# nlesc-smcm/hymls

Measured on AMD Instinct MI355X. Metric: Preconditioner ApplyInverse DoF/s + achieved HBM GB/s, Stokes3D, higher is better.
Workload: dtype f64

## Files before the change

### hymls_amd/csrc/device.hpp

```cpp
#pragma once
#include <cstdio>
#include "common.hpp"
#include "symbolic.hpp"

namespace hymls {
namespace dev {

struct Context;
Context* create_context(int device);
void bind(Context* c);
Context* current();
void destroy_context(Context* c);
void* stream();
const double* zeros16();
void* alloc(size_t bytes);
void free(void* p);
void h2d(void* dst, const void* src, size_t bytes);
void d2h(void* dst, const void* src, size_t bytes);
void d2d(void* dst, const void* src, size_t bytes);
void zero(void* dst, size_t bytes);
void sync();
size_t mem_free();
void* shared_scratch(size_t bytes);
constexpr int NSIDE = 8;
// ... 52 lines not shown
  const int32_t* fw_ptr;
  const int32_t* fw_items;
  const struct FwRec* fw_rec;
  const int32_t* bw_ptr;
  const int32_t* bw_items;
  int32_t nlev, max_level_rows;
  int32_t s_ent_begin, s_ent_end;
  int64_t scratch_size, factor_size;
  int32_t contrib_size;
  int32_t max_solve_rows;
  int32_t packed;
};

struct BatchD {
  int32_t nb;
  const int32_t* src;
  const int32_t* xoff;
  double* factor;
  double* scratch;
  double* sblock;
  double* contrib;
  int32_t* flag;
  double* tmp;
  int64_t tmp_stride;
  double* swork;
  int64_t swork_stride;
};

void gather(int64_t n, const int32_t* idx, const double* src, double* dst);
void scatter(int64_t n, const int32_t* idx, const double* src, double* dst);
void scatter_add(int64_t n, const int32_t* idx, const double* src, double* dst);
void axpby(int64_t n, double a, const double* x, double b, double* y);
void scale_copy(int64_t n, double a, const double* x, double* y);
void spmv(int32_t nrows, const int32_t* rowptr, const int32_t* col, const double* val,
          const double* x, double* y, double alpha, double beta, int64_t nnz_hint = -1);
void pull_sum(int64_t n, const int64_t* ptr, const int64_t* idx, const double* in, double* out);
void offdiag_count(int64_t nrows, const int32_t* rows, const int32_t* krow, const int32_t* kcol, const int32_t* ta, const int32_t* tb,
                   const int32_t* excl, int32_t* count);
void offdiag_fill(int64_t nrows, const int32_t* rows, const int32_t* krow, const int32_t* kcol, const int32_t* ta, const int32_t* tb,
                  const int32_t* excl, const int32_t* rowptr, int32_t* col, int32_t* src);
void member_sources(int32_t nb, int32_t next, int32_t nent, const int32_t* ext, const int32_t* ent_row, const int32_t* ent_col,
                    const int32_t* krow, const int32_t* kcol, int32_t* src, int32_t* flag);
void build_pull_tables(int64_t nrows, const int64_t* rcount, const int32_t* rowptr, const uint64_t* keys, int64_t* ptr, int64_t* idx);
void pull_sum_blocks(int64_t blen, int32_t nblk, const int64_t* ptr, const int64_t* base,
                     const double* in, double* out);

void factor_level(const PlanD& P, const BatchD& B, const int32_t* list, int32_t count,
                  int32_t b0, int32_t nbc, const double* kval, int32_t max_w);
void sblock_init(const PlanD& P, const BatchD& B, int32_t b0, int32_t nbc, const double* kval);

constexpr int PIECE = 128;
void factor_big_front(const PlanD& P, const BatchD& B, const FrontD& F, const FrontD* kids, int32_t nkids,
                      int32_t b0, int32_t nbc, const double* kval);
void root_update(const PlanD& P, const BatchD& B, const FrontD& F, int32_t nbc);
inline int solve_kt() {
  static const int kt = (std::getenv("HYMLS_MI_SOLVE_KT") && std::atoi(std::getenv("HYMLS_MI_SOLVE_KT")) == 1024) ? 1024 : 256;
  return kt;
}
void solve_fwd_big(const PlanD& P, const BatchD& B, const int32_t* list, const FrontD* hfronts, const int64_t* poff,
                   int32_t count, double* x);
void solve_bwd_big(const PlanD& P, const BatchD& B, const int32_t* list, const FrontD* hfronts, const int64_t* poff,
                   int32_t count, double* x);

void solve_fwd_level(const PlanD& P, const BatchD& B, const int32_t* list, int32_t count, double* x);
void solve_bwd_level(const PlanD& P, const BatchD& B, const int32_t* list, int32_t count, double* x);

#if defined(__HIPCC__)
#define HYMLS_HD __host__ __device__
#else
#define HYMLS_HD
#endif
HYMLS_HD inline int64_t packed_lower(int64_t w, int64_t i, int64_t k) { return k * (2 * w - k - 1) / 2 + (i - k - 1); }
HYMLS_HD inline int64_t packed_l21(int64_t w, int64_t ri, int64_t i, int64_t k) { return w * (w - 1) / 2 + i + ri * k; }
HYMLS_HD inline int64_t packed_upper(int64_t w, int64_t ri, int64_t i, int64_t k) { return w * (w - 1) / 2 + ri * w + k * (k + 1) / 2 + i; }
void repack_fronts(const PlanD& P, const BatchD& B, int32_t b0, int32_t nbc);

struct FusedSub {
  union {
    const double* fac;
    const float* fac32;
  };
  int32_t xoff;
  int32_t cls;
};
constexpr int FUSED_MAX_ITEMS = 2048;
struct FusedIO {
  int32_t in = 0, out = 0;
  const double* b = nullptr; const int32_t* perm = nullptr;
  const int32_t* a_row = nullptr; const int32_t* a_col = nullptr; const double* a_val = nullptr; const double* x2 = nullptr;
  const double* z = nullptr; double* user = nullptr;
};
void interior_solve_fused(int32_t nsub, const FusedSub* subs, const PlanD* plans, int32_t lds_doubles, double* x,
                          const FusedIO* io = nullptr);

constexpr int32_t FLAG_F32_RANGE = 4;
void demote_panels(int64_t n, const double* src, float* dst, int32_t* flag);
void round_panels(int64_t n, double* slab, int32_t* flag);
void interior_solve_fused_f32(int32_t nsub, const FusedSub* subs, const PlanD* plans, int32_t lds_doubles, double* x,
                              const FusedIO* io = nullptr);

struct LvlSub { const double* fac; double* contrib; int32_t xoff, cls; int64_t cstride; };
struct LvlTask { int32_t sub, front, r0, pad; };
constexpr int LVL_MAX_ROWS = 6144;
constexpr int LVL_SMALL_ROWS = 256;
void solve_fwd_tasks(const LvlTask* tasks, int32_t ntasks, const LvlSub* subs, const PlanD* plans, int32_t lds_doubles,
                     const double* x, double* y);
void solve_bwd_tasks(const LvlTask* tasks, int32_t ntasks, const LvlSub* subs, const PlanD* plans, int32_t lds_doubles,
                     const double* y, double* x);

constexpr int NV_MAX = 4;
void interior_solve_fused_mv(int32_t nsub, const FusedSub* subs, const PlanD* plans, int32_t lds_doubles, int32_t front_doubles,
                             double* x, int64_t ldx, int nv);
void interior_solve_fused_mv_f32(int32_t nsub, const FusedSub* subs, const PlanD* plans, int32_t lds_doubles, int32_t front_doubles,
                                 double* x, int64_t ldx, int nv);
void solve_fwd_tasks_mv(const LvlTask* tasks, int32_t ntasks, const LvlSub* subs, const PlanD* plans, int32_t lds_doubles,
                        const double* x, double* y, int64_t ld, int nv);
void solve_bwd_tasks_mv(const LvlTask* tasks, int32_t ntasks, const LvlSub* subs, const PlanD* plans, int32_t lds_doubles,
                        const double* y, double* x, int64_t ld, int nv);

void ot_apply(int32_t ng, const int32_t* gptr, const double* w, double* x);
// ... 26 lines not shown
```

### hymls_amd/csrc/device_hip.hip

```cpp
#include <hip/hip_runtime.h>
#include <type_traits>
#include <dlfcn.h>
#include <chrono>
#include <cstring>
#include <cfloat>
#include <array>
#include <map>
#include <string>
#include <cstdio>
#include "device.hpp"

namespace hymls {
namespace dev {

#define HIP_CHECK(call)                                                                    \
  do {                                                                                     \
    hipError_t e_ = (call);                                                                \
    if (e_ != hipSuccess)                                                                  \
      throw ::hymls::Error(-3, std::string("HIP error: ") + hipGetErrorString(e_) + " at " + \
                                   __FILE__ + ":" + std::to_string(__LINE__));             \
  } while (0)

struct MarkRec { int phase; bool begin; hipEvent_t ev; };
struct Context {
// ... 263 lines not shown
  if (n <= 0) return;
  hipLaunchKernelGGL(k_scatter_add, dim3(nblocks(n, 256, 65536)), dim3(256), 0, g_stream, n, idx, src, dst); launch_check();
}
void axpby(int64_t n, double a, const double* x, double b, double* y) {
  if (n <= 0) return;
  hipLaunchKernelGGL(k_axpby, dim3(nblocks(n, 256, 8192)), dim3(256), 0, g_stream, n, a, x, b, y); launch_check();
}
void scale_copy(int64_t n, double a, const double* x, double* y) {
  if (n <= 0) return;
  hipLaunchKernelGGL(k_scale_copy, dim3(nblocks(n, 256, 8192)), dim3(256), 0, g_stream, n, a, x, y); launch_check();
}

template <int L>
__global__ void k_spmv(int32_t nrows, const int32_t* __restrict__ rp, const int32_t* __restrict__ col,
                       const double* __restrict__ val, const double* __restrict__ x, double* __restrict__ y,
                       double alpha, double beta) {
  const int lane = (int)(threadIdx.x % L);
  const int rpb = (int)blockDim.x / L;
  for (int64_t base = (int64_t)blockIdx.x * rpb; base < nrows; base += (int64_t)gridDim.x * rpb) {
    const int64_t row = base + threadIdx.x / L;
    double s = 0.0;
    if (row < nrows) {
      const int b = rp[row], e = rp[row + 1];
      for (int k = b + lane; k < e; k += L) s += val[k] * x[col[k]];
    }
#pragma unroll
    for (int off = L / 2; off > 0; off >>= 1) s += __shfl_down(s, off, L);
    if (row < nrows && lane == 0) y[row] = alpha * s + (beta == 0.0 ? 0.0 : beta * y[row]);
  }
}
void spmv(int32_t nrows, const int32_t* rp, const int32_t* col, const double* val, const double* x, double* y,
          double alpha, double beta, int64_t nnz_hint) {
  if (nrows <= 0) return;
  const double avg = nnz_hint >= 0 ? (double)nnz_hint / nrows : 8.0;
  const int L = avg < 2.5 ? 1 : (avg < 5.0 ? 2 : (avg < 20.0 ? 4 : 8));
  const int64_t nt = (int64_t)nrows * L;
  const dim3 grid(nblocks(nt, 256));
  switch (L) {
    case 1: hipLaunchKernelGGL(k_spmv<1>, grid, dim3(256), 0, g_stream, nrows, rp, col, val, x, y, alpha, beta); break;
    case 2: hipLaunchKernelGGL(k_spmv<2>, grid, dim3(256), 0, g_stream, nrows, rp, col, val, x, y, alpha, beta); break;
    case 4: hipLaunchKernelGGL(k_spmv<4>, grid, dim3(256), 0, g_stream, nrows, rp, col, val, x, y, alpha, beta); break;
    default: hipLaunchKernelGGL(k_spmv<8>, grid, dim3(256), 0, g_stream, nrows, rp, col, val, x, y, alpha, beta); break;
  }
  launch_check();
}

__global__ void k_pull_sum(int64_t n, const int64_t* __restrict__ ptr, const int64_t* __restrict__ idx,
                           const double* __restrict__ in, double* __restrict__ out) {
  for (int64_t e = blockIdx.x * (int64_t)blockDim.x + threadIdx.x; e < n; e += (int64_t)gridDim.x * blockDim.x) {
    double s = 0.0;
    for (int64_t t = ptr[e]; t < ptr[e + 1]; t++) s += in[idx[t]];
    out[e] = s;
  }
}
void pull_sum(int64_t n, const int64_t* ptr, const int64_t* idx, const double* in, double* out) {
  if (n <= 0) return;
  hipLaunchKernelGGL(k_pull_sum, dim3(nblocks(n, 256, 65536)), dim3(256), 0, g_stream, n, ptr, idx, in, out); launch_check();
}
template <bool FILL>
__global__ void __launch_bounds__(256) k_offdiag(int64_t nrows, const int32_t* __restrict__ rows, const int32_t* __restrict__ krow,
                                                 const int32_t* __restrict__ kcol, const int32_t* __restrict__ ta, const int32_t* __restrict__ tb,
                                                 const int32_t* __restrict__ excl, const int32_t* __restrict__ rowptr, int32_t* __restrict__ out,
                                                 int32_t* __restrict__ src) {
  for (int64_t t = blockIdx.x * (int64_t)blockDim.x + threadIdx.x; t < nrows; t += (int64_t)gridDim.x * blockDim.x) {
    const int32_t r = rows[t];
    int32_t o = FILL ? rowptr[t] : 0;
    for (int32_t e = krow[r]; e < krow[r + 1]; e++) {
      const int32_t c = kcol[e];
// ... 1625 lines not shown
  if ((uintptr_t)(src + head) % 16 != 0) head = n;
  hipLaunchKernelGGL(k_demote_panels, dim3(nblocks(std::max<int64_t>(n / 4, 1), 256, 8192)), dim3(256), 0, g_stream, src, dst, n, head, flag);
  launch_check();
}
__global__ void __launch_bounds__(256) k_round_panels(double* __restrict__ slab, int64_t n, int32_t* __restrict__ flag) {
  bool bad = false;
  for (int64_t t = (int64_t)blockIdx.x * 256 + threadIdx.x; t < n; t += (int64_t)gridDim.x * 256) {
    const double v = slab[t];
    bad |= !(fabs(v) <= (double)FLT_MAX);
    slab[t] = (double)(float)v;
  }
  if (bad) atomicOr(flag, FLAG_F32_RANGE);
}
void round_panels(int64_t n, double* slab, int32_t* flag) {
  if (n <= 0) return;
  hipLaunchKernelGGL(k_round_panels, dim3(nblocks(n, 256, 8192)), dim3(256), 0, g_stream, slab, n, flag);
  launch_check();
}

struct FusedFront { int32_t c0, w, ri, c_off, a_off, lf_off, idx_off, pad; int64_t lp_off, q_off; };
template <class PTR>
__device__ inline PTR lside(PTR base, int packed, int r, int w, int ri, int& c1, int& tri) {
  if (!packed) { c1 = w + ri; tri = 0; return base + r; }
  if (r < w) { c1 = w; tri = 1; return base + (r - 1); }
  c1 = ri; tri = 0;
  return base + ((w * (w - 1)) >> 1) + (r - w);
}
template <class PTR>
__device__ inline PTR uside(PTR base, int packed, int i, int w, int ri, int& c1, int& tri) {
  if (!packed) { c1 = w + ri; tri = 0; return base + i; }
  c1 = 0; tri = 1;
  return base + ((w * (w - 1)) >> 1) + ri * w + i;
}
template <bool PROF, class PT>
__global__ void __launch_bounds__(256) __attribute__((amdgpu_waves_per_eu(8, 8))) k_interior_fused(const FusedSub* __restrict__ subs, const PlanD* __restrict__ plans,
                                                         double* __restrict__ x, long long* __restrict__ prof, FusedIO io) {
  extern __shared__ double lds[];
  auto ldp = [](gptr<PT> q) { return (double)*q; };
  long long tp[6] = {0, 0, 0, 0, 0, 0}, t0 = 0, tstart = 0;
  auto tick = [&](int bucket) { if (PROF) { const long long t = wall_clock64(); tp[bucket] += t - t0; t0 = t; } };
  if (PROF) { t0 = wall_clock64(); tstart = t0; }
  const FusedSub S = subs[blockIdx.x];
  const PlanD P = plans[S.cls];
  double* X = lds;
  double* C = lds + P.nI;
  double* Fv = C + P.contrib_size;
  double* R = Fv + 128;
  FusedFront* LF = (FusedFront*)(Fv + (P.max_level_rows > 384 ? P.max_level_rows : 384));
  const int tid = threadIdx.x;
  for (int i = tid; i < P.nfronts; i += 256) {
    const FrontD G = P.fronts[i];
    FusedFront f;
    f.c0 = G.c0; f.w = G.w; f.ri = G.ri; f.c_off = G.c_off; f.a_off = G.a_off; f.lf_off = G.lf_off; f.idx_off = G.idx_off; f.pad = 0;
    f.lp_off = G.lp_off; f.q_off = G.q_off;
    LF[i] = f;
  }
  double* xg = x + S.xoff;
  if (io.in == 0) {
    for (int i = tid; i < P.nI; i += 256) X[i] = xg[i];
  } else if (io.in == 1) {
    for (int i = tid; i < P.nI; i += 256) X[i] = io.b[io.perm[S.xoff + i]];
  } else {
    for (int i = tid; i < P.nI; i += 256) {
      double v = 0.0;
      for (int e = io.a_row[S.xoff + i]; e < io.a_row[S.xoff + i + 1]; e++) v += io.a_val[e] * io.x2[io.a_col[e]];
      X[i] = v;
    }
  }
  __syncthreads();
  tick(0);
  const gptr<PT> fac = as_global((const PT*)(const void*)S.fac);
  const gptr<int32_t> fw_items = as_global(P.fw_items), bw_items = as_global(P.bw_items), fidx = as_global(P.fidx),
                      asm_ptr = as_global(P.asm_ptr), asm_src = as_global(P.asm_src), fw_ptr = as_global(P.fw_ptr), bw_ptr = as_global(P.bw_ptr);
  typedef int v4i __attribute__((ext_vector_type(4)));
  const gptr<v4i> fw_rec = (gptr<v4i>)P.fw_rec;
  for (int lev = 0; lev < P.nlev; lev++) {
    const int ib = fw_ptr[lev], ni = fw_ptr[lev + 1] - ib;
    for (int it = tid; it < ni; it += 256) {
      FwRec rc;
      { const v4i q = fw_rec[ib + it]; static_assert(sizeof(FwRec) == 16, "FwRec is one dwordx4"); __builtin_memcpy(&rc, &q, 16); }
      const int item = rc.item;
      const FusedFront& F = LF[item >> 16];
      const int r = item & 0xffff;
      double v = r < F.w ? X[F.c0 + r] : 0.0;
      if (rc.n != 0xffff) {
#pragma unroll
        for (int q = 0; q < 5; q++) if (q < rc.n) v += C[rc.s[q]];
      } else {
        for (int t = asm_ptr[F.a_off + r]; t < asm_ptr[F.a_off + r + 1]; t++) v += C[asm_src[t]];
      }
      if (r < F.w) Fv[F.lf_off + r] = v; else C[F.c_off + r - F.w] = v;
    }
    __syncthreads();
    tick(1);
    if (ni > 128) {
      for (int it = tid; it < ni; it += 256) {
        const int item = fw_items[ib + it];
        const FusedFront& F = LF[item >> 16];
        const int r = item & 0xffff, w = F.w;
// ... 100 lines not shown
        const int i = item & 0xffff, w = F.w, ri = F.ri;
        int c1, tri;
        const gptr<PT> p = uside(fac + F.lp_off, P.packed, i, w, ri, c1, tri);
        const double* Xs = X + F.c0;
        auto at = [&](int kk) { return ldp(p + (c1 * kk + tri * ((kk * (kk + 1)) >> 1))); };
        int k = i + kg;
        for (; k + 3 * KG < w; k += 4 * KG) {
          const double l0 = at(k), l1 = at(k + KG), l2 = at(k + 2 * KG), l3 = at(k + 3 * KG);
          a0 += l0 * Xs[k]; a1 += l1 * Xs[k + KG]; a2 += l2 * Xs[k + 2 * KG]; a3 += l3 * Xs[k + 3 * KG];
        }
        for (; k < w; k += KG) a0 += at(k) * Xs[k];
        const gptr<PT> qv = fac + F.q_off + i;
        const gptr<int32_t> idx = fidx + F.idx_off + w;
        k = kg;
        for (; k + 3 * KG < ri; k += 4 * KG) {
          const double q0 = ldp(qv + (int64_t)w * k), q1 = ldp(qv + (int64_t)w * (k + KG)), q2 = ldp(qv + (int64_t)w * (k + 2 * KG)), q3 = ldp(qv + (int64_t)w * (k + 3 * KG));
          const int i0 = idx[k], i1 = idx[k + KG], i2 = idx[k + 2 * KG], i3 = idx[k + 3 * KG];
          a0 -= q0 * X[i0]; a1 -= q1 * X[i1]; a2 -= q2 * X[i2]; a3 -= q3 * X[i3];
        }
        for (; k < ri; k += KG) a0 -= ldp(qv + (int64_t)w * k) * X[idx[k]];
      }
      R[kg * RT + it] = (a0 + a1) + (a2 + a3);
      __syncthreads();
      if (tid < ni) {
        const int item = bw_items[ib + tid];
        double sum = 0.0;
        for (int g = 0; g < KG; g++) sum += R[g * RT + tid];
        X[LF[item >> 16].c0 + (item & 0xffff)] = sum;
      }
    }
    __syncthreads();
    tick(ni > 128 ? 3 : 4);
  }
  if (io.out == 0) {
    for (int i = tid; i < P.nI; i += 256) xg[i] = X[i];
  } else {
    for (int i = tid; i < P.nI; i += 256) io.user[io.perm[S.xoff + i]] = io.z[S.xoff + i] - X[i];
  }
  if (PROF && tid == 0) {
    tp[5] = wall_clock64() - tstart;
    for (int q = 0; q < 6; q++) prof[(int64_t)blockIdx.x * 8 + q] = tp[q];
    prof[(int64_t)blockIdx.x * 8 + 6] = tstart;
    prof[(int64_t)blockIdx.x * 8 + 7] = P.nI;
  }
}

template <class PT>
static void launch_fused(int32_t nsub, const FusedSub* subs, const PlanD* plans, int32_t lds_doubles, double* x, const FusedIO* iop) {
  const FusedIO io = iop ? *iop : FusedIO();
  if (nsub <= 0) return;
  const size_t shm = (size_t)lds_doubles * sizeof(double);
  if (std::getenv("HYMLS_MI_FUSED_PROF")) {
    long long* dprof = (long long*)alloc((size_t)nsub * 8 * sizeof(long long));
    if (shm > 64 * 1024) HIP_CHECK(hipFuncSetAttribute((const void*)k_interior_fused<true, PT>, hipFuncAttributeMaxDynamicSharedMemorySize, (int)shm));
    hipLaunchKernelGGL((k_interior_fused<true, PT>), dim3(nsub), dim3(256), shm, g_stream, subs, plans, x, dprof, io);
    launch_check();
    std::vector<long long> h((size_t)nsub * 8);
    d2h(h.data(), dprof, h.size() * sizeof(long long));
    free(dprof);
    double sum[6] = {0, 0, 0, 0, 0, 0};
    long long tmin = h[6], tmax = 0;
    for (int b = 0; b < nsub; b++) { for (int q = 0; q < 6; q++) sum[q] += (double)h[(size_t)b * 8 + q]; tmin = std::min(tmin, h[(size_t)b * 8 + 6]); tmax = std::max(tmax, h[(size_t)b * 8 + 6] + h[(size_t)b * 8 + 5]); }
    std::fprintf(stderr, "[hymls_mi] fused solve: %d workgroups, kernel span %.1f us; mean per workgroup (us): setup %.1f | fwd assembly %.1f | fwd panels %.1f | bwd panels (wide levels) %.1f | bwd panels (k-split levels) %.1f | total %.1f\n",
                 nsub, (tmax - tmin) / 100.0, sum[0] / nsub / 100, sum[1] / nsub / 100, sum[2] / nsub / 100, sum[3] / nsub / 100, sum[4] / nsub / 100, sum[5] / nsub / 100);
    return;
  }
  if (shm > 64 * 1024) HIP_CHECK(hipFuncSetAttribute((const void*)k_interior_fused<false, PT>, hipFuncAttributeMaxDynamicSharedMemorySize, (int)shm));
  hipLaunchKernelGGL((k_interior_fused<false, PT>), dim3(nsub), dim3(256), shm, g_stream, subs, plans, x, (long long*)nullptr, io);
  launch_check();
}
void interior_solve_fused(int32_t nsub, const FusedSub* subs, const PlanD* plans, int32_t lds_doubles, double* x, const FusedIO* iop) {
  launch_fused<double>(nsub, subs, plans, lds_doubles, x, iop);
}
void interior_solve_fused_f32(int32_t nsub, const FusedSub* subs, const PlanD* plans, int32_t lds_doubles, double* x, const FusedIO* iop) {
  launch_fused<float>(nsub, subs, plans, lds_doubles, x, iop);
}

constexpr size_t LDS_LIMIT_BYTES = 160 * 1024;
static int mv_group_cap(const char* which) {
  const char* e = std::getenv((std::string("HYMLS_MI_MV_GROUP_") + which).c_str());
  return e ? std::max(1, std::atoi(e)) : NV_MAX;
}

template <int NV, class PT>
__global__ void __launch_bounds__(256) k_interior_fused_mv(const FusedSub* __restrict__ subs, const PlanD* __restrict__ plans,
                                                            double* __restrict__ x, int64_t ldx) {
  extern __shared__ double lds[];
  const FusedSub S = subs[blockIdx.x];
  const PlanD P = plans[S.cls];
  const int nI = P.nI, CS = P.contrib_size, FS = P.max_level_rows > 384 ? P.max_level_rows : 384;
  double* X = lds;
  double* C = X + NV * nI;
  double* Fv = C + NV * CS;
  FusedFront* LF = (FusedFront*)(Fv + NV * FS);
  const int tid = threadIdx.x;
  for (int i = tid; i < P.nfronts; i += 256) {
    const FrontD G = P.fronts[i];
    FusedFront f;
    f.c0 = G.c0; f.w = G.w; f.ri = G.ri; f.c_off = G.c_off; f.a_off = G.a_off; f.lf_off = G.lf_off; f.idx_off = G.idx_off; f.pad = 0;
    f.lp_off = G.lp_off; f.q_off = G.q_off;
    LF[i] = f;
  }
// ... 1203 lines not shown
```

### hymls_amd/csrc/precond.cpp

```cpp
#include "precond.hpp"
#include <cstring>
#include <chrono>
#include <thread>
#include <mutex>
#include <atomic>
#include <map>
#include <unordered_map>

namespace hymls {

namespace {

struct Hasher {
  uint64_t h = 1469598103934665603ULL;
  void add(const void* p, size_t n) {
    const unsigned char* c = (const unsigned char*)p;
    size_t i = 0;
    for (; i + 8 <= n; i += 8) {
      uint64_t w;
      std::memcpy(&w, c + i, 8);
      h = (h ^ w) * 0x9E3779B97F4A7C15ULL;
      h ^= h >> 29;
    }
    for (; i < n; i++) { h ^= c[i]; h *= 1099511628211ULL; }
// ... 926 lines not shown
      dev::offdiag_fill(nr, d_rows, d_krow_, d_kcol_, ta, tb, excl, d_row, d_col, d_src);
      col.resize(nz); src.resize(nz);
      if (nz) { dev::d2h(col.data(), d_col, nz * sizeof(int32_t)); dev::d2h(src.data(), d_src, nz * sizeof(int32_t)); }
    };
    cut(n1_, d_rows1, d_pos2, nullptr, nullptr, a12_row_, a12_col_, a12_src_, d_a12_row_, d_a12_col_, d_a12_src_);
    fine("A12 count / prefix / fill (device)");
    cut(n2_, d_rows2, d_int, d_ghost, d_pos2, a21_row_, a21_col_, a21_src_, d_a21_row_, d_a21_col_, d_a21_src_);
    dev::sync();
    dev::free(d_pos2); dev::free(d_int); dev::free(d_ghost); dev::free(d_rows1); dev::free(d_rows2);
  }
  if (dist) {
    xch_int_.build(*comm_, want_int, dst_int, [&](int64_t g) { const int l = g2l_[g]; return l >= 0 ? intidx_[l] : -1; });
    xch_sep_.build(*comm_, want_sep, dst_sep, [&](int64_t g) { const int l = g2l_[g]; return (l >= 0 && pos2_[l] < n2_) ? pos2_[l] : -1; });
  }
  fine("A21 count / prefix / fill + halo plans");
  lap("A12/A21 + halo plans");
  for (auto& cp : cls_) {
    const size_t fb = BatchedLU::factor_bytes((int64_t)cp->lu.members.size(), cp->lu.plan.factor_size);
    if (fb >= ((size_t)1 << 30) && !cp->lu.pre_factor) cp->lu.pre_factor.reset(new AsyncAlloc(fb));
  }
  for (auto& cp : cls_) { cp->lu.d_krow = d_krow_; cp->lu.d_kcol = d_kcol_; }
  build_schur_setup();
  lap("Schur setup + uploads");
  d_kval_ = (double*)dev::alloc(std::max<size_t>(1, K_.val.size()) * sizeof(double));
  d_inperm_ = dev::upload(in_perm_);
  d_z_ = (double*)dev::alloc((size_t)std::max(n1_ + ngi_ + n2_, 1) * sizeof(double));
  d_t1_ = (double*)dev::alloc((size_t)std::max(n1_, 1) * sizeof(double));
  d_t2_ = (double*)dev::alloc((size_t)std::max(n2_ + ngs_, 1) * sizeof(double));
  d_y2_ = (double*)dev::alloc((size_t)std::max(n2_, 1) * sizeof(double));
  d_yb_ = (double*)dev::alloc((size_t)std::max(n2_, 1) * sizeof(double));
  d_a12_val_ = (double*)dev::alloc(std::max<size_t>(1, a12_col_.size()) * sizeof(double));
  d_a21_val_ = (double*)dev::alloc(std::max<size_t>(1, a21_col_.size()) * sizeof(double));
  d_flag_ = (int32_t*)dev::alloc(sizeof(int32_t));
  initialized_ = true;
}

void LevelSolver::build_classes() {
  const bool verbose_bc = std::getenv("HYMLS_MI_VERBOSE") != nullptr && (level_ == 0 || std::atoi(std::getenv("HYMLS_MI_VERBOSE")) >= 2);
  double t_bc = wall();
  auto lap_bc = [&](const char* what) {
    if (!verbose_bc) return;
    std::fprintf(stderr, "[hymls_mi] rank %d level %d:   classes / %-22s %.2f s\n", comm_->rank, level_, what, wall() - t_bc);
    t_bc = wall();
  };
  const int n = K_.n;
  const int nsd = (int)hm_.sd.size();
  const int nsep = n2_ + ngs_;
  auto sidx = [&](int32_t gid) { const int l = g2l_[gid]; return l >= 0 ? pos2_[l] : -1; };
  ivec cnt(nsep + 1, 0);
  for (auto& S : hm_.sd) for (auto& g : S.groups) for (int32_t x : g.nodes) { const int k = sidx(x); if (k >= 0) cnt[k + 1]++; }
  for (int i = 0; i < nsep; i++) cnt[i + 1] += cnt[i];
  ivec sdl(cnt[nsep]), fill(cnt.begin(), cnt.end() - 1);
  for (int s = 0; s < nsd; s++)
    for (auto& g : hm_.sd[s].groups) for (int32_t x : g.nodes) { const int k = sidx(x); if (k >= 0) sdl[fill[k]++] = s; }
  auto common = [&](int a, int b) {
    int c = 0, i = cnt[a], j = cnt[b];
    const int ie = cnt[a + 1], je = cnt[b + 1];
    while (i < ie && j < je) {
      const int x = sdl[i], y = sdl[j];
      c += x == y; i += x <= y; j += y <= x;
    }
    return c;
  };
  FineLap fine;
  sep_sd_ptr_ = cnt; sep_sd_ = sdl;
  fine("(classes) subdomains listing each separator node");
// ... 1086 lines not shown
      parallel_assign(next_pattern_key_col_, R.col.data(), R.col.size());
      fnl("(next level) pattern key copy");
      next_level_ = new LevelSolver(p_.next_level(), level_ + 1, ngid_, comm_);
      next_.reset(next_level_);
      next_level_->set_rows(R, next_gids, glob_tv_, R.n);
      fnl("(next level) set_rows");
      next_level_->initialize();
      fnl("(next level) initialize");
      build_handoff(next_level_->owned_gids());
      fnl("(next level) hand-off");
    }
    next_level_->profiling = false;
    lap("next level initialize");
    set_next_border();
    next_level_->set_factor_bits(factor_bits_);
    next_level_->compute();
    lap("next level compute");
  } else {
    DirectSolver* ds = next_is_direct_ && !next_level_ ? dynamic_cast<DirectSolver*>(next_.get()) : nullptr;
    if (!(ds && ds->refactor(R, next_gids, p_.fix_gid, p_, bm_ > 0))) {
      next_.reset();
      next_level_ = nullptr;
      next_is_direct_ = true;
      next_.reset(new DirectSolver(R, next_gids, p_.fix_gid, ngid_, p_, &glob_clu_ptr_, &glob_clu_, &glob_sd_center_, bm_ > 0));
      build_handoff(next_gids);
    }
    set_next_border();
    lap("coarse solver");
  }
}

void LevelSolver::interior_solve(double* x1) { interior_solve_mv(x1, n1_ + ngi_, 1); }

void LevelSolver::interior_solve_mv(double* x1, int64_t ld, int nv) {
  dev::Range range("MatrixBlock", level_ + 1, "ApplyInverse");
  if (n_fsubs_ > 0) {
#ifdef HYMLS_MI_F32_PANELS
    if (fsubs_bits_ == 32) {
      if (nv == 1) dev::interior_solve_fused_f32(n_fsubs_, d_fsubs_, d_fplans_, fused_lds_, x1);
      else dev::interior_solve_fused_mv_f32(n_fsubs_, d_fsubs_, d_fplans_, fused_vec_lds_ + fused_front_lds_, fused_front_lds_, x1, ld, nv);
    } else
#endif
    if (nv == 1) dev::interior_solve_fused(n_fsubs_, d_fsubs_, d_fplans_, fused_lds_, x1);
    else dev::interior_solve_fused_mv(n_fsubs_, d_fsubs_, d_fplans_, fused_vec_lds_ + fused_front_lds_, fused_front_lds_, x1, ld, nv);
  }
  if (merged_.nsubs > 0) {
    ensure_nvec(nv);
    merged_.solve(d_fplans_, x1, d_ytmp_, ld, nv);
  }
  for (size_t c = 0; c < cls_.size(); c++)
    if (!cls_fused_[c] && !cls_merged_[c])
      for (int v = 0; v < nv; v++) cls_[c]->lu.solve(x1 + v * ld);
}

void LevelSolver::ensure_nvec(int nv) {
  if (nv <= nvec_alloc_) return;
  dev::sync();
  auto grow = [&](double*& p, int64_t len) { dev::free(p); p = (double*)dev::alloc((size_t)std::max<int64_t>(len, 1) * nv * sizeof(double)); };
  grow(d_z_, n1_ + ngi_ + n2_); grow(d_t1_, n1_); grow(d_t2_, n2_ + ngs_);
  if (!direct_schur_) { const int64_t ng = (int64_t)vs_.size(); grow(d_vrhs_, ng); grow(d_vsol_, ng); }
  if (d_nrhs_) { grow(d_nrhs_, n_next_owned_); grow(d_nsol_, n_next_owned_); }
  if (d_ytmp_) grow(d_ytmp_, n1_ + ngi_ + n2_);
  nvec_alloc_ = nv;
}

void LevelSolver::next_apply(const double* rhs, double* sol, int64_t ld, int nv) {
  if (!comm_->distributed()) { next_->apply_inverse_mv(rhs, ld, sol, ld, nv); return; }
  const int64_t ldn = std::max<int64_t>(n_next_owned_, 1);
  for (int v = 0; v < nv; v++) xch_down_.forward(rhs + v * ld, d_nrhs_ + v * ldn);
  next_->apply_inverse_mv(d_nrhs_, ldn, d_nsol_, ldn, nv);
  for (int v = 0; v < nv; v++) {
    if (next_is_direct_) {
      if (red_.n) dev::d2d(sol + v * ld, d_nsol_ + v * ldn + glob_row_off_[comm_->rank], (size_t)red_.n * sizeof(double));
    } else {
      xch_down_.backward(d_nsol_ + v * ldn, sol + v * ld);
    }
// ... 1 lines not shown
}

void LevelSolver::schur_apply(double* rhs2, int64_t ldr, double* x2, int64_t ldx, int nv) {
  dev::Range range("SchurPreconditioner", level_ + 1, "ApplyInverse");
  if (global_n2_ == 0) return;
  if (direct_schur_) {
    if (!comm_->distributed()) { next_->apply_inverse_mv(rhs2, ldr, x2, ldx, nv); return; }
    for (int v = 0; v < nv; v++) next_apply(rhs2 + v * ldr, x2 + v * ldx, 0, 1);
    return;
  }
  const int ng = (int)vs_.size();
  const int64_t ldv = std::max(ng, 1);
  for (int v = 0; v < nv; v++) dev::ot_apply(ng, d_gptr_, d_otw_, rhs2 + v * ldr);
  dev::blocks_apply_all_mv(n_blk_apply_, d_blka_, blk_max_nb_, rhs2, ldr, x2, ldx, nv);
  for (int v = 0; v < nv; v++) dev::gather(ng, d_vs_, rhs2 + v * ldr, d_vrhs_ + v * ldv);
  if (profiling && level_ == 0) dev::mark(4, true);
  next_apply(d_vrhs_, d_vsol_, ldv, nv);
  if (profiling && level_ == 0) dev::mark(4, false);
  for (int v = 0; v < nv; v++) {
    dev::scatter(ng, d_vs_, d_vsol_ + v * ldv, x2 + v * ldx);
    dev::ot_apply(ng, d_gptr_, d_otw_, x2 + v * ldx);
  }
}

void LevelSolver::apply_inverse(const double* b, double* x) { apply_inverse_mv(b, 0, x, 0, 1); }

void LevelSolver::apply_inverse_mv(const double* b, int64_t ldb, double* x, int64_t ldx, int nv) {
  dev::Range range("Preconditioner", level_ + 1, "ApplyInverse");
  HYMLS_CHECK(next_ != nullptr || global_n2_ == 0, -1, "The preconditioner has not yet been computed.");
  ensure_nvec(nv);
  const int64_t ldz = n1_ + ngi_ + n2_, ld1 = std::max(n1_, 1), ld2 = std::max(n2_ + ngs_, 1);
  double* z1 = d_z_;
  double* z2 = d_z_ + n1_ + ngi_;
  if (profiling) dev::mark(0, true);
  for (int v = 0; v < nv; v++) {
    dev::gather(n1_, d_inperm_, b + v * ldb, z1 + v * ldz);
    dev::gather(n2_, d_inperm_ + n1_, b + v * ldb, z2 + v * ldz);
  }
  if (profiling) dev::mark(1, true);
  interior_solve_mv(z1, ldz, nv);
  if (profiling) { dev::mark(1, false); dev::mark(2, true); }
  for (int v = 0; v < nv; v++) {
    xch_int_.forward(z1 + v * ldz, z1 + v * ldz);
    dev::spmv(n2_, d_a21_row_, d_a21_col_, d_a21_val_, z1 + v * ldz, z2 + v * ldz, -1.0, 1.0, (int64_t)a21_col_.size());
  }
  if (profiling) { dev::mark(2, false); dev::mark(3, true); }
  schur_apply(z2, ldz, d_t2_, ld2, nv);
  if (profiling) { dev::mark(3, false); dev::mark(2, true); }
  for (int v = 0; v < nv; v++) {
    xch_sep_.forward(d_t2_ + v * ld2, d_t2_ + v * ld2);
    dev::spmv(n1_, d_a12_row_, d_a12_col_, d_a12_val_, d_t2_ + v * ld2, d_t1_ + v * ld1, 1.0, 0.0, (int64_t)a12_col_.size());
  }
  if (profiling) { dev::mark(2, false); dev::mark(1, true); }
  interior_solve_mv(d_t1_, ld1, nv);
  if (profiling) dev::mark(1, false);
  for (int v = 0; v < nv; v++) {
    dev::axpby(n1_, -1.0, d_t1_ + v * ld1, 1.0, z1 + v * ldz);
    dev::scatter(n1_, d_inperm_, z1 + v * ldz, x + v * ldx);
    dev::scatter(n2_, d_inperm_ + n1_, d_t2_ + v * ld2, x + v * ldx);
  }
  if (profiling) dev::mark(0, false);
}

void LevelSolver::build_matvec() {
  const int n = K_.n, nown = (int)owned_gids_.size();
  ivec user(n, -1);
  {
    int u = 0;
    for (int i = 0; i < nrows_; i++) if (intidx_[i] >= 0 || (pos2_[i] >= 0 && pos2_[i] < n2_)) user[i] = u++;
  }
  ivec row(1, 0), col, src, node(nown);
  std::vector<char> wanted(n, 0);
  ivec want;
  for (int i = 0; i < nrows_; i++) {
    if (user[i] < 0) continue;
    node[user[i]] = i;
    for (int e = K_.rowptr[i]; e < K_.rowptr[i + 1]; e++) {
      const int c = K_.col[e];
      col.push_back(c); src.push_back(e);
      if (user[c] < 0 && !wanted[c]) { wanted[c] = 1; want.push_back(gids_[c]); }
    }
// ... 198 lines not shown
  xch_sep_.forward(d_t2_, d_t2_);
  dev::spmv(n1_, d_a12_row_, d_a12_col_, d_a12_val_, d_t2_, d_t1_, 1.0, 0.0);
  interior_solve(d_t1_);
  dev::axpby(n1_, -1.0, d_t1_, 1.0, z1);
  for (int j = 0; j < m; j++) dev::axpby(n1_, -S[j], d_bQ1_ + (size_t)j * (n1_ + ngi_), 1.0, z1);
  dev::scatter(n1_, d_inperm_, z1, x);
  dev::scatter(n2_, d_inperm_ + n1_, d_t2_, x);
}

void LevelSolver::matvec(const double* x, double* y) {
  dev::Range range("MatrixBlock", level_ + 1, "Apply");
  if (!comm_->distributed()) { dev::spmv(K_.n, d_krow_, d_kcol_, d_kval_, x, y, 1.0, 0.0); return; }
  if (!mv_ready_) build_matvec();
  if (mv_stale_) { dev::gather(mv_nnz_, d_mv_src_, d_kval_, d_mv_val_); mv_stale_ = false; }
  const int nown = (int)owned_gids_.size();
  dev::scatter(nown, d_mv_node_, x, d_mv_x_);
  xch_mv_.forward(x, d_mv_x_);
  dev::spmv(nown, d_mv_row_, d_mv_col_, d_mv_val_, d_mv_x_, y, 1.0, 0.0);
}

void LevelSolver::add_stats(ApplyStats& st, bool as_coarse) const {
  double f = 0, fs = 0, sp = 0, sep = 0, vec = 0;
  for (auto& cp : cls_) {
    f += 2.0 * (cp->lu.factor32 ? 4.0 : 8.0) * (double)cp->lu.plan.nnz_factor * (double)cp->lu.members.size();
    st.bytes_resident += cp->lu.resident_bytes();
    fs += 2.0 * (12.0 * (double)cp->lu.plan.nnz_sparse + 24.0 * cp->lu.plan.nI) * (double)cp->lu.members.size();
  }
  sp = 12.0 * (double)(a12_col_.size() + a21_col_.size()) + 4.0 * (n1_ + n2_ + 2);
  if (!direct_schur_) {
    sep = 2.0 * 12.0 * n2_;
    for (auto& B : blocks_) sep += (8.0 * B.nb * B.nb + 4.0 * B.nb) * B.nblk;
  }
  const double N = (double)(n1_ + n2_);
  vec = 8.0 * (4.0 * N + 7.0 * n1_ + 12.0 * n2_);
  for (auto& cp : cls_) {
    st.flops_factor += (double)cp->lu.plan.flops_factor * (double)cp->lu.members.size();
    if (!direct_schur_) st.flops_transform += 4.0 * (double)cp->pat.nS * (double)cp->pat.nS * (double)cp->lu.members.size();
  }
  if (!direct_schur_) for (auto& B : blocks_) st.flops_blocks += 2.0 * (double)B.nb * B.nb * B.nb * B.nblk;
  if (as_coarse) { st.bytes_coarse += f + sp + sep + vec; st.bytes_coarse_sparse += fs + sp + sep + vec; }
  else { st.bytes_factor += f; st.bytes_factor_sparse += fs; st.bytes_spmv += sp; st.bytes_sep += sep; st.bytes_vec += vec; }
  if (next_) next_->add_stats(st, true);
}

}
```

### hymls_amd/csrc/precond.hpp

```cpp
#pragma once
#include <memory>
#include <thread>
#include <exception>
#include "common.hpp"
#include "partition.hpp"
#include "symbolic.hpp"
#include "device.hpp"
#include "comm.hpp"

namespace hymls {

struct ApplyStats {
  double bytes_factor = 0, bytes_spmv = 0, bytes_sep = 0, bytes_coarse = 0, bytes_vec = 0;
  double bytes_factor_sparse = 0, bytes_coarse_sparse = 0;
  double flops_factor = 0, flops_blocks = 0, flops_transform = 0;
  double bytes_resident = 0;
};

struct AsyncAlloc {
  std::thread th;
  void* p = nullptr;
  size_t bytes = 0;
  std::exception_ptr err;
  explicit AsyncAlloc(size_t n) : bytes(n) {
// ... 150 lines not shown
  void apply_inverse_mv(const double* b, int64_t ldb, double* x, int64_t ldx, int nv) override;
  void set_border(int m, const double* dV, const double* dW, const double* C) override;
  void apply_inverse_bordered(const double* b, const double* T, double* x, double* S) override;
  bool have_border() const { return bm_ > 0; }
  void set_factor_bits(int bits) { factor_bits_ = bits; }
  int border_size() const { return bm_; }
  int64_t size() const override { return global_n_; }
  void add_stats(ApplyStats& st, bool as_coarse) const override;
  void matvec(const double* x, double* y);

  const HierMap& hiermap() const { return hm_; }
  int level() const { return level_; }
  int64_t schur_size() const { return global_n2_; }
  int64_t num_subdomains_global() const { return (int64_t)hm_.sd.size(); }
  const ivec& owned_gids() const { return owned_gids_; }
  int64_t num_owned() const { return (int64_t)owned_gids_.size(); }
  int32_t num_rows() const { return nrows_; }
  Operator* next() const { return next_.get(); }
  LevelSolver* next_level() const { return next_level_; }
  double phase_seconds[5] = {0, 0, 0, 0, 0};
  bool profiling = false;

 private:
  struct Cls;
  struct ExtLayout { int32_t ngl = 0; std::vector<int64_t> blk_off; ivec blk_len; int64_t size = 0; };
  ExtLayout ext_layout(const Subdomain& S) const;
  void localize();
  void build_classes();
  void build_schur_setup();
  void exchange_records();
  const Csr& assemble_reduced(ivec& row_gids, dvec* tvn);
  void schur_apply(double* rhs2, int64_t ldr, double* x2, int64_t ldx, int nv);
  void next_apply(const double* rhs, double* sol, int64_t ld, int nv);
  void interior_solve_mv(double* x1, int64_t ld, int nv);
  void ensure_nvec(int nv);
  int nvec_alloc_ = 1;
  void build_handoff(const ivec& next_owned);
  void interior_solve(double* x1);
  void interior_solve_transposed(double* x1);
  void compute_border();
  void set_next_border();
  void schur_apply_bordered(double* rhs2, const double* q, double* x2, double* S);
  void next_apply_bordered(const double* rhs, const double* T, double* sol, double* S);
  int64_t n_next_owned_ = 0;
  int bm_ = 0;
  dvec bC_, bSC_;
  double *d_bVu_ = nullptr, *d_bWu_ = nullptr;
  double *d_bW1_ = nullptr, *d_bQ1_ = nullptr, *d_bSV_ = nullptr, *d_bSW_ = nullptr, *d_bNV_ = nullptr, *d_bNW_ = nullptr, *d_btmp_ = nullptr;
  int32_t *d_a12t_row_ = nullptr, *d_a12t_col_ = nullptr, *d_a12t_src_ = nullptr;
  double* d_a12t_val_ = nullptr;
  int64_t a12t_nnz_ = 0;
  std::vector<int32_t*> d_orders_;
  ivec order_rows_;

  Params p_;
  int level_;
  int64_t ngid_;
  const Comm* comm_;
  Csr K_;
  int32_t nrows_ = 0;
  ivec keep_entries_;
  size_t given_nnz_ = 0;
  ivec gids_;
  dvec tv_;
  HierMap hm_;
  bool partitioned_ = false;
  ivec sd_rank_;
  ivec my_sds_, halo_sds_;
  int64_t global_n_ = 0, global_n2_ = 0;
  int32_t n1_ = 0, n2_ = 0, ngs_ = 0, ngi_ = 0;
  ivec g2l_;
  ivec sep_row_;
  ivec pos2_;
  ivec intidx_;
  ivec in_perm_;
  ivec owned_gids_;
  ivec sd_xoff_, sd_cls_, sd_bidx_;
  ivec sep_sd_ptr_, sep_sd_;
  ivec sd_center_;
  std::vector<std::unique_ptr<Cls>> cls_;
  Exchange xch_int_, xch_sep_, xch_down_, xch_mv_;
  bool mv_ready_ = false, mv_stale_ = true;
  int32_t *d_mv_row_ = nullptr, *d_mv_col_ = nullptr, *d_mv_src_ = nullptr, *d_mv_node_ = nullptr;
  double *d_mv_val_ = nullptr, *d_mv_x_ = nullptr;
  int64_t mv_nnz_ = 0;
  void build_matvec();
  struct RecSeg { int64_t off, len; };
  std::vector<RecSeg> rec_send_;
  std::vector<int64_t> rec_scnt_, rec_rcnt_;
  int64_t rec_nsend_ = 0, rec_nrecv_ = 0, ext_recv_base_ = 0;
  bool rec_any_ = false;
  dev::FusedSub* d_fsubs_ = nullptr;
  dev::PlanD* d_fplans_ = nullptr;
  int32_t n_fsubs_ = 0, fused_lds_ = 0, fused_front_lds_ = 0, fused_vec_lds_ = 0;
  std::vector<char> cls_fused_;
  int factor_bits_ = 64;
  int fsubs_bits_ = 64;
  void prepare_factor_storage();
  void finish_factor_storage();
  std::vector<char> cls_merged_;
  MergedSolve merged_;
  double* d_ytmp_ = nullptr;
  double* d_kval_ = nullptr;
  int32_t *d_krow_ = nullptr, *d_kcol_ = nullptr;
  int32_t* d_inperm_ = nullptr;
  double *d_z_ = nullptr, *d_t1_ = nullptr, *d_t2_ = nullptr, *d_y2_ = nullptr;
  ivec a12_row_, a21_row_;
  cvec a12_col_, a12_src_, a21_col_, a21_src_;
  int32_t *d_a12_row_ = nullptr, *d_a12_col_ = nullptr, *d_a12_src_ = nullptr;
  int32_t *d_a21_row_ = nullptr, *d_a21_col_ = nullptr, *d_a21_src_ = nullptr;
  double *d_a12_val_ = nullptr, *d_a21_val_ = nullptr;
  bool direct_schur_ = false;
  ivec gptr_;
  dvec otw_;
  ivec vs_;
  int32_t* d_gptr_ = nullptr; double* d_otw_ = nullptr; int32_t* d_vs_ = nullptr;
  struct BlockClass { int32_t nb = 0, nblk = 0; ivec ids; ivec owner_key; double* d_binv = nullptr; int32_t* d_ids = nullptr;
                      std::vector<int64_t> pull_ptr, pull_base; int64_t* d_pull_ptr = nullptr; int64_t* d_pull_base = nullptr; };
  std::vector<BlockClass> blocks_;
  dev::BlkD* d_blkd_ = nullptr;
  dev::BlkD* d_blka_ = nullptr;
  int32_t n_blk_ = 0, n_blk_apply_ = 0, blk_max_nb_ = 0, blk_max_nb_inv_ = 0;
  Csr red_;
  int64_t n_pulls_ = 0;
  int64_t *d_red_pull_ptr_ = nullptr, *d_red_pull_idx_ = nullptr;
  double* d_red_val_ = nullptr;
  double* d_ext_ = nullptr; int64_t ext_total_ = 0;
  double *d_vrhs_ = nullptr, *d_vsol_ = nullptr, *d_yb_ = nullptr;
// ... 23 lines not shown
```

Measured before the change: 2.384 billion.

## Fuse input gather and A12 spmv/output scatter into fused interior solve kernel

When the fused per-subdomain classes cover every interior row, the apply folds the gather of b into the first interior solve and folds the A12 spmv, the z minus x subtraction and the permuted scatter into the second interior solve. The IO modes become template parameters with separate kernel instantiations, and the in-kernel spmv uses a lane-parallel row reduction. This is meant to remove several separate vector passes and kernel launches over the interior unknowns. The cost is more kernel variants, more register and code pressure in the fused kernel, and a gate that only applies for single-vector applies with no merged subdomains.

```diff
diff --git a/hymls_amd/csrc/device.hpp b/hymls_amd/csrc/device.hpp
--- a/hymls_amd/csrc/device.hpp
+++ b/hymls_amd/csrc/device.hpp
@@ -108,6 +108,10 @@
 void scatter_add(int64_t n, const int32_t* idx, const double* src, double* dst);
 void axpby(int64_t n, double a, const double* x, double b, double* y);
 void scale_copy(int64_t n, double a, const double* x, double* y);
+inline int spmv_lanes(int32_t nrows, int64_t nnz_hint) {
+  const double avg = nnz_hint >= 0 ? (double)nnz_hint / nrows : 8.0;
+  return avg < 2.5 ? 1 : (avg < 5.0 ? 2 : (avg < 20.0 ? 4 : 8));
+}
 void spmv(int32_t nrows, const int32_t* rowptr, const int32_t* col, const double* val,
           const double* x, double* y, double alpha, double beta, int64_t nnz_hint = -1);
 void pull_sum(int64_t n, const int64_t* ptr, const int64_t* idx, const double* in, double* out);
@@ -161,7 +165,7 @@
 };
 constexpr int FUSED_MAX_ITEMS = 2048;
 struct FusedIO {
-  int32_t in = 0, out = 0;
+  int32_t in = 0, out = 0, a_lanes = 1;
   const double* b = nullptr; const int32_t* perm = nullptr;
   const int32_t* a_row = nullptr; const int32_t* a_col = nullptr; const double* a_val = nullptr; const double* x2 = nullptr;
   const double* z = nullptr; double* user = nullptr;
diff --git a/hymls_amd/csrc/device_hip.hip b/hymls_amd/csrc/device_hip.hip
--- a/hymls_amd/csrc/device_hip.hip
+++ b/hymls_amd/csrc/device_hip.hip
@@ -319,8 +319,7 @@
 void spmv(int32_t nrows, const int32_t* rp, const int32_t* col, const double* val, const double* x, double* y,
           double alpha, double beta, int64_t nnz_hint) {
   if (nrows <= 0) return;
-  const double avg = nnz_hint >= 0 ? (double)nnz_hint / nrows : 8.0;
-  const int L = avg < 2.5 ? 1 : (avg < 5.0 ? 2 : (avg < 20.0 ? 4 : 8));
+  const int L = spmv_lanes(nrows, nnz_hint);
   const int64_t nt = (int64_t)nrows * L;
   const dim3 grid(nblocks(nt, 256));
   switch (L) {
@@ -2012,9 +2011,24 @@
   c1 = 0; tri = 1;
   return base + ((w * (w - 1)) >> 1) + ri * w + i;
 }
-template <bool PROF, class PT>
-__global__ void __launch_bounds__(256) __attribute__((amdgpu_waves_per_eu(8, 8))) k_interior_fused(const FusedSub* __restrict__ subs, const PlanD* __restrict__ plans,
-                                                         double* __restrict__ x, long long* __restrict__ prof, FusedIO io) {
+template <int L>
+__device__ __forceinline__ void fused_spmv_rows(int n, int tid, gptr<int32_t> rp, gptr<int32_t> col, gptr<double> val, gptr<double> x, double* y) {
+  const int lane = tid % L, rpb = 256 / L;
+  for (int base = 0; base < n; base += rpb) {
+    const int row = base + tid / L;
+    double s = 0.0;
+    if (row < n) {
+      const int b = rp[row], e = rp[row + 1];
+      for (int k = b + lane; k < e; k += L) s += val[k] * x[col[k]];
+    }
+#pragma unroll
+    for (int off = L / 2; off > 0; off >>= 1) s += __shfl_down(s, off, L);
+    if (row < n && lane == 0) y[row] = s + 0.0;
+  }
+}
+template <bool PROF, class PT, int IN, int OUT>
+__device__ __forceinline__ void interior_fused_body(const FusedSub* __restrict__ subs, const PlanD* __restrict__ plans,
+                                                    double* __restrict__ x, long long* __restrict__ prof, const FusedIO io) {
   extern __shared__ double lds[];
   auto ldp = [](gptr<PT> q) { return (double)*q; };
   long long tp[6] = {0, 0, 0, 0, 0, 0}, t0 = 0, tstart = 0;
@@ -2036,15 +2050,20 @@
     LF[i] = f;
   }
   double* xg = x + S.xoff;
-  if (io.in == 0) {
+  if (IN == 0) {
     for (int i = tid; i < P.nI; i += 256) X[i] = xg[i];
-  } else if (io.in == 1) {
-    for (int i = tid; i < P.nI; i += 256) X[i] = io.b[io.perm[S.xoff + i]];
+  } else if (IN == 1) {
+    const gptr<int32_t> perm = as_global(io.perm) + S.xoff;
+    const gptr<double> b = as_global(io.b);
+    for (int i = tid; i < P.nI; i += 256) X[i] = b[perm[i]];
   } else {
-    for (int i = tid; i < P.nI; i += 256) {
-      double v = 0.0;
-      for (int e = io.a_row[S.xoff + i]; e < io.a_row[S.xoff + i + 1]; e++) v += io.a_val[e] * io.x2[io.a_col[e]];
-      X[i] = v;
+    const gptr<int32_t> a_row = as_global(io.a_row) + S.xoff, a_col = as_global(io.a_col);
+    const gptr<double> a_val = as_global(io.a_val), x2 = as_global(io.x2);
+    switch (io.a_lanes) {
+      case 1: fused_spmv_rows<1>(P.nI, tid, a_row, a_col, a_val, x2, X); break;
+      case 2: fused_spmv_rows<2>(P.nI, tid, a_row, a_col, a_val, x2, X); break;
+      case 4: fused_spmv_rows<4>(P.nI, tid, a_row, a_col, a_val, x2, X); break;
+      default: fused_spmv_rows<8>(P.nI, tid, a_row, a_col, a_val, x2, X); break;
     }
   }
   __syncthreads();
@@ -2211,10 +2230,13 @@
     __syncthreads();
     tick(ni > 128 ? 3 : 4);
   }
-  if (io.out == 0) {
+  if (OUT == 0) {
     for (int i = tid; i < P.nI; i += 256) xg[i] = X[i];
   } else {
-    for (int i = tid; i < P.nI; i += 256) io.user[io.perm[S.xoff + i]] = io.z[S.xoff + i] - X[i];
+    const gptr<int32_t> perm = as_global(io.perm) + S.xoff;
+    const gptr<double> z = as_global(io.z) + S.xoff;
+    const gmptr<double> user = as_global_rw(io.user);
+    for (int i = tid; i < P.nI; i += 256) user[perm[i]] = z[i] - X[i];
   }
   if (PROF && tid == 0) {
     tp[5] = wall_clock64() - tstart;
@@ -2223,17 +2245,38 @@
     prof[(int64_t)blockIdx.x * 8 + 7] = P.nI;
   }
 }
-
+template <bool PROF, class PT>
+__global__ void __launch_bounds__(256) __attribute__((amdgpu_waves_per_eu(8, 8))) k_interior_fused(const FusedSub* __restrict__ subs, const PlanD* __restrict__ plans,
+                                                         double* __restrict__ x, long long* __restrict__ prof) {
+  interior_fused_body<PROF, PT, 0, 0>(subs, plans, x, prof, FusedIO());
+}
+template <bool PROF, class PT, int IN, int OUT>
+__global__ void __launch_bounds__(256) __attribute__((amdgpu_waves_per_eu(8, 8))) k_interior_fused_io(const FusedSub* __restrict__ subs, const PlanD* __restrict__ plans,
+                                                            double* __restrict__ x, long long* __restrict__ prof, FusedIO io) {
+  interior_fused_body<PROF, PT, IN, OUT>(subs, plans, x, prof, io);
+}
+
+template <bool PROF, class PT>
+static void launch_fused_kernel(int32_t nsub, const FusedSub* subs, const PlanD* plans, size_t shm, double* x, long long* prof, const FusedIO& io) {
+  auto go = [&](auto kernel, auto... tail) {
+    if (shm > 64 * 1024) HIP_CHECK(hipFuncSetAttribute((const void*)kernel, hipFuncAttributeMaxDynamicSharedMemorySize, (int)shm));
+    hipLaunchKernelGGL(kernel, dim3(nsub), dim3(256), shm, g_stream, subs, plans, x, prof, tail...);
+  };
+  if (io.in == 0 && io.out == 0) go(k_interior_fused<PROF, PT>);
+  else if (io.in == 1 && io.out == 0) go(k_interior_fused_io<PROF, PT, 1, 0>, io);
+  else if (io.in == 2 && io.out == 1) go(k_interior_fused_io<PROF, PT, 2, 1>, io);
+  else HYMLS_CHECK(false, -3, "fused interior solve: no kernel for this combination of FusedIO::in and FusedIO::out");
+  launch_check();
+}
 template <class PT>
 static void launch_fused(int32_t nsub, const FusedSub* subs, const PlanD* plans, int32_t lds_doubles, double* x, const FusedIO* iop) {
   const FusedIO io = iop ? *iop : FusedIO();
   if (nsub <= 0) return;
   const size_t shm = (size_t)lds_doubles * sizeof(double);
-  if (std::getenv("HYMLS_MI_FUSED_PROF")) {
+  static const bool phase_prof = std::getenv("HYMLS_MI_FUSED_PROF") != nullptr;
+  if (phase_prof) {
     long long* dprof = (long long*)alloc((size_t)nsub * 8 * sizeof(long long));
-    if (shm > 64 * 1024) HIP_CHECK(hipFuncSetAttribute((const void*)k_interior_fused<true, PT>, hipFuncAttributeMaxDynamicSharedMemorySize, (int)shm));
-    hipLaunchKernelGGL((k_interior_fused<true, PT>), dim3(nsub), dim3(256), shm, g_stream, subs, plans, x, dprof, io);
-    launch_check();
+    launch_fused_kernel<true, PT>(nsub, subs, plans, shm, x, dprof, io);
     std::vector<long long> h((size_t)nsub * 8);
     d2h(h.data(), dprof, h.size() * sizeof(long long));
     free(dprof);
@@ -2244,9 +2287,7 @@
                  nsub, (tmax - tmin) / 100.0, sum[0] / nsub / 100, sum[1] / nsub / 100, sum[2] / nsub / 100, sum[3] / nsub / 100, sum[4] / nsub / 100, sum[5] / nsub / 100);
     return;
   }
-  if (shm > 64 * 1024) HIP_CHECK(hipFuncSetAttribute((const void*)k_interior_fused<false, PT>, hipFuncAttributeMaxDynamicSharedMemorySize, (int)shm));
-  hipLaunchKernelGGL((k_interior_fused<false, PT>), dim3(nsub), dim3(256), shm, g_stream, subs, plans, x, (long long*)nullptr, io);
-  launch_check();
+  launch_fused_kernel<false, PT>(nsub, subs, plans, shm, x, nullptr, io);
 }
 void interior_solve_fused(int32_t nsub, const FusedSub* subs, const PlanD* plans, int32_t lds_doubles, double* x, const FusedIO* iop) {
   launch_fused<double>(nsub, subs, plans, lds_doubles, x, iop);
diff --git a/hymls_amd/csrc/precond.cpp b/hymls_amd/csrc/precond.cpp
--- a/hymls_amd/csrc/precond.cpp
+++ b/hymls_amd/csrc/precond.cpp
@@ -982,6 +982,15 @@
   d_a12_val_ = (double*)dev::alloc(std::max<size_t>(1, a12_col_.size()) * sizeof(double));
   d_a21_val_ = (double*)dev::alloc(std::max<size_t>(1, a21_col_.size()) * sizeof(double));
   d_flag_ = (int32_t*)dev::alloc(sizeof(int32_t));
+  {
+    int64_t covered = 0;
+    for (size_t c = 0; c < cls_.size(); c++)
+      if (cls_fused_[c]) covered += (int64_t)cls_[c]->lu.plan.nI * (int64_t)cls_[c]->lu.members.size();
+    fused_io_ = n1_ > 0 && covered == n1_ && merged_.nsubs == 0 && !std::getenv("HYMLS_MI_NO_FUSED_IO");
+    if (std::getenv("HYMLS_MI_VERBOSE"))
+      std::fprintf(stderr, "[hymls_mi] rank %d level %d: vector passes of the apply %s the interior solve (fused classes cover %lld of %d interior rows, A12 %.2f entries per row)\n",
+                   comm_->rank, level_, fused_io_ ? "fused into" : "separate from", (long long)covered, n1_, n1_ ? (double)a12_col_.size() / n1_ : 0.0);
+  }
   initialized_ = true;
 }
 
@@ -2134,16 +2143,17 @@
 
 void LevelSolver::interior_solve(double* x1) { interior_solve_mv(x1, n1_ + ngi_, 1); }
 
-void LevelSolver::interior_solve_mv(double* x1, int64_t ld, int nv) {
+void LevelSolver::interior_solve_mv(double* x1, int64_t ld, int nv, const dev::FusedIO* io) {
   dev::Range range("MatrixBlock", level_ + 1, "ApplyInverse");
+  HYMLS_CHECK(io == nullptr || (fused_io_ && nv == 1), -3, "fused vector passes need the fused interior solve of one vector");
   if (n_fsubs_ > 0) {
 #ifdef HYMLS_MI_F32_PANELS
     if (fsubs_bits_ == 32) {
-      if (nv == 1) dev::interior_solve_fused_f32(n_fsubs_, d_fsubs_, d_fplans_, fused_lds_, x1);
+      if (nv == 1) dev::interior_solve_fused_f32(n_fsubs_, d_fsubs_, d_fplans_, fused_lds_, x1, io);
       else dev::interior_solve_fused_mv_f32(n_fsubs_, d_fsubs_, d_fplans_, fused_vec_lds_ + fused_front_lds_, fused_front_lds_, x1, ld, nv);
     } else
 #endif
-    if (nv == 1) dev::interior_solve_fused(n_fsubs_, d_fsubs_, d_fplans_, fused_lds_, x1);
+    if (nv == 1) dev::interior_solve_fused(n_fsubs_, d_fsubs_, d_fplans_, fused_lds_, x1, io);
     else dev::interior_solve_fused_mv(n_fsubs_, d_fsubs_, d_fplans_, fused_vec_lds_ + fused_front_lds_, fused_front_lds_, x1, ld, nv);
   }
   if (merged_.nsubs > 0) {
@@ -2211,13 +2221,20 @@
   const int64_t ldz = n1_ + ngi_ + n2_, ld1 = std::max(n1_, 1), ld2 = std::max(n2_ + ngs_, 1);
   double* z1 = d_z_;
   double* z2 = d_z_ + n1_ + ngi_;
+  const bool fio = fused_io_ && nv == 1;
   if (profiling) dev::mark(0, true);
   for (int v = 0; v < nv; v++) {
-    dev::gather(n1_, d_inperm_, b + v * ldb, z1 + v * ldz);
+    if (!fio) dev::gather(n1_, d_inperm_, b + v * ldb, z1 + v * ldz);
     dev::gather(n2_, d_inperm_ + n1_, b + v * ldb, z2 + v * ldz);
   }
   if (profiling) dev::mark(1, true);
-  interior_solve_mv(z1, ldz, nv);
+  if (fio) {
+    dev::FusedIO io;
+    io.in = 1; io.b = b; io.perm = d_inperm_;
+    interior_solve_mv(z1, ldz, 1, &io);
+  } else {
+    interior_solve_mv(z1, ldz, nv);
+  }
   if (profiling) { dev::mark(1, false); dev::mark(2, true); }
   for (int v = 0; v < nv; v++) {
     xch_int_.forward(z1 + v * ldz, z1 + v * ldz);
@@ -2225,7 +2242,21 @@
   }
   if (profiling) { dev::mark(2, false); dev::mark(3, true); }
   schur_apply(z2, ldz, d_t2_, ld2, nv);
-  if (profiling) { dev::mark(3, false); dev::mark(2, true); }
+  if (profiling) dev::mark(3, false);
+  if (fio) {
+    xch_sep_.forward(d_t2_, d_t2_);
+    if (profiling) dev::mark(1, true);
+    dev::FusedIO io;
+    io.in = 2; io.a_row = d_a12_row_; io.a_col = d_a12_col_; io.a_val = d_a12_val_; io.x2 = d_t2_;
+    io.a_lanes = dev::spmv_lanes(n1_, (int64_t)a12_col_.size());
+    io.out = 1; io.z = z1; io.user = x; io.perm = d_inperm_;
+    interior_solve_mv(d_t1_, ld1, 1, &io);
+    if (profiling) dev::mark(1, false);
+    dev::scatter(n2_, d_inperm_ + n1_, d_t2_, x);
+    if (profiling) dev::mark(0, false);
+    return;
+  }
+  if (profiling) dev::mark(2, true);
   for (int v = 0; v < nv; v++) {
     xch_sep_.forward(d_t2_ + v * ld2, d_t2_ + v * ld2);
     dev::spmv(n1_, d_a12_row_, d_a12_col_, d_a12_val_, d_t2_ + v * ld2, d_t1_ + v * ld1, 1.0, 0.0, (int64_t)a12_col_.size());
@@ -2490,7 +2521,7 @@
     for (auto& B : blocks_) sep += (8.0 * B.nb * B.nb + 4.0 * B.nb) * B.nblk;
   }
   const double N = (double)(n1_ + n2_);
-  vec = 8.0 * (4.0 * N + 7.0 * n1_ + 12.0 * n2_);
+  vec = 8.0 * (4.0 * N + (fused_io_ ? 0.0 : 7.0) * n1_ + 12.0 * n2_);
   for (auto& cp : cls_) {
     st.flops_factor += (double)cp->lu.plan.flops_factor * (double)cp->lu.members.size();
     if (!direct_schur_) st.flops_transform += 4.0 * (double)cp->pat.nS * (double)cp->pat.nS * (double)cp->lu.members.size();
diff --git a/hymls_amd/csrc/precond.hpp b/hymls_amd/csrc/precond.hpp
--- a/hymls_amd/csrc/precond.hpp
+++ b/hymls_amd/csrc/precond.hpp
@@ -206,7 +206,7 @@
   const Csr& assemble_reduced(ivec& row_gids, dvec* tvn);
   void schur_apply(double* rhs2, int64_t ldr, double* x2, int64_t ldx, int nv);
   void next_apply(const double* rhs, double* sol, int64_t ld, int nv);
-  void interior_solve_mv(double* x1, int64_t ld, int nv);
+  void interior_solve_mv(double* x1, int64_t ld, int nv, const dev::FusedIO* io = nullptr);
   void ensure_nvec(int nv);
   int nvec_alloc_ = 1;
   void build_handoff(const ivec& next_owned);
@@ -268,6 +268,7 @@
   dev::PlanD* d_fplans_ = nullptr;
   int32_t n_fsubs_ = 0, fused_lds_ = 0, fused_front_lds_ = 0, fused_vec_lds_ = 0;
   std::vector<char> cls_fused_;
+  bool fused_io_ = false;
   int factor_bits_ = 64;
   int fsubs_bits_ = 64;
   void prepare_factor_storage();
```

Result: faster. 2.439 billion, median of 6 (+2.3%).
